# ChristophReich1996/Multi-StyleGAN

Measured on AMD Instinct MI355X. Metric: training images/sec (G+D step, 256^2, seq=3x2ch), higher is better.
Workload: dtype bf16

## Files before the change

### include/msg_hip.h

```cpp
#ifndef MSG_HIP_H
#define MSG_HIP_H

#ifdef __cplusplus
extern "C" {
#endif

enum { MSG_OK = 0, MSG_EINVAL = -1, MSG_EUNSUPPORTED = -2, MSG_ELAUNCH = -3 };
enum { MSG_F32 = 0, MSG_BF16 = 1, MSG_F16 = 2, MSG_F64 = 3, MSG_F32_SPLIT = 4 };

#define MSG_ABI_VERSION 5
int msg_abi_version(void);
const char* msg_build_arch(void);
const char* msg_strerror(int code);

int msg_upfirdn2d(const void* x, const float* fir, void* y, int dtype,
                  int major, int in_h, int in_w, int minor, int kh, int kw,
                  int up_x, int up_y, int down_x, int down_y,
                  int pad_x0, int pad_x1, int pad_y0, int pad_y1, void* stream);

int msg_upfirdn2d_pitched(const void* x, const float* fir, void* y, int dtype,
                          int major, int in_h, int in_w, int minor, int in_pitch, int kh, int kw,
                          int up_x, int up_y, int down_x, int down_y,
                          int pad_x0, int pad_x1, int pad_y0, int pad_y1, void* stream);

int msg_upfirdn2d_pitched2(const void* x, const float* fir, void* y, int dtype,
                           int major, int in_h, int in_w, int minor, int in_pitch, int out_pitch, int kh, int kw,
                           int up_x, int up_y, int down_x, int down_y,
                           int pad_x0, int pad_x1, int pad_y0, int pad_y1, void* stream);

int msg_upfirdn2d_separable(const void* x, const float* fir_y, const float* fir_x, void* y, int dtype,
                            int major, int in_h, int in_w, int minor, int kh, int kw,
                            int pad_x0, int pad_x1, int pad_y0, int pad_y1, void* stream);

int msg_upfirdn2d_separable_act(const void* x, const float* fir_y, const float* fir_x, void* y, int dtype,
                                int major, int in_h, int in_w, int minor, int kh, int kw,
                                int pad_x0, int pad_x1, int pad_y0, int pad_y1,
                                const float* act_bias, const float* noise, const float* noise_weight,
                                int noise_batch, float alpha, float scale, void* stream);
int msg_upfirdn2d_separable_act_mask(const void* x, const float* fir_y, const float* fir_x, void* y, int dtype,
                                     int major, int in_h, int in_w, int minor, int kh, int kw,
                                     int pad_x0, int pad_x1, int pad_y0, int pad_y1,
                                     const float* act_bias, const float* noise, const float* noise_weight,
                                     int noise_batch, float alpha, float scale, unsigned char* mask, void* stream);

int msg_fused_bias_act(const void* x, const float* bias, const void* ref, void* y, int dtype,
                       long long size_x, int step_b, int size_b,
                       const float* noise, const float* noise_weight, int noise_batch, int pix,
                       int act, int grad, float alpha, float scale, void* stream);

long long msg_bias_act_backward_workspace(long long size_x, int step_b, int size_b, int has_noise);
int msg_bias_act_backward(const void* gy, const void* out, void* gx, int dtype,
                          long long size_x, int step_b, int size_b,
                          float* grad_bias, const float* noise, float* grad_noise_weight,
                          int noise_batch, int pix, float alpha, float scale,
                          float* ws, long long ws_floats, void* stream);
int msg_channel_sums(const void* x, float* sums, int dtype, long long size_x, int C, float* ws, long long ws_floats,
                     void* stream);
int msg_bias_act_backward_mask(const void* gy, const unsigned char* mask, int tile_m, int tile_n, void* gx, int dtype,
                               long long size_x, int size_b,
                               float* grad_bias, const float* noise, float* grad_noise_weight,
                               int noise_batch, int pix, float alpha, float scale,
                               float* ws, long long ws_floats, void* stream);
int msg_sum_rows(const float* part, float* out, long long rows, int cols, void* stream);
int msg_bias_act_backward_mask_head(const void* gy, const void* ghead, const float* whead, const float* style,
                                    float wscale, int n_head, const unsigned char* mask, int tile_m, int tile_n,
                                    void* gx, int dtype, long long size_x, int size_b,
                                    float* grad_bias, const float* noise, float* grad_noise_weight,
                                    int noise_batch, int pix, float alpha, float scale,
                                    float* ws, long long ws_floats, void* stream);

int msg_conv2d_fprop(const void* x, const void* w, const float* bias, void* y, int dtype,
                     int B, int IH, int IW, int Cx, int Ck, int OH, int OW, int N, int ldy,
                     int kh, int kw, int stride, int pad, int in_up, int pixel_shuffle,
                     long long w_batch_stride, void* stream);
enum { MSG_WGRAD_K_AUTO = -1 };
int msg_conv2d_wgrad(const void* gy, const void* x, float* gw, int dtype,
                     int B, int IH, int IW, int Cx, int I, int OH, int OW, int ldgy, int O, int ldgw,
                     int kh, int kw, int stride, int pad, int pixel_shuffle,
                     int per_sample, int k_chunks, int oi_major, float gain,
                     float* ws, long long ws_floats, void* stream);
long long msg_conv2d_wgrad_workspace(int dtype, int B, int IH, int IW, int Cx, int I, int OH, int OW, int ldgy,
                                     int O, int ldgw, int kh, int kw, int stride, int pad, int pixel_shuffle,
                                     int per_sample, int k_chunks);

int msg_demod_coeff(const float* W, const float* s, float* d, int B, int O, int I, int taps,
                    float scale, float eps, void* stream);
int msg_scale_rows_cols(const float* base, const float* rowscale, const float* colscale, void* out,
                        int dtype, int B, int R, int T, int C, int Ck, float gain, void* stream);
int msg_modulate_weights(const float* base, const float* wsq, const float* style, void* out, float* d_out,
                         int dtype, int B, int R, int O, int T, int C, int Ck, float scale, float eps, void* stream);
int msg_modulate_backward(const float* gwk, const float* W, const float* s, const float* d, float* gW,
                          float* gs_part, int B, int O, int I, int taps, int ldg, int o_group,
                          float scale, void* stream);
int msg_scale_rows_cols2(const float* base, const float* row1, const float* col1, const float* row2, const float* col2,
                         void* out, int dtype, int B, int R, int T, int C, int Ck, float gain, void* stream);
int msg_modulate_backward2(const float* gwk, const float* W, const float* s, const float* d, const float* v,
                           float* gW, float* gs_part, int B, int O, int I, int taps, int ldg, int o_group,
                           float scale, void* stream);

int msg_relayout_weight(const float* w, void* fwd, void* dgrad, float* wsq, int dtype,
                        int O, int I, int T, int Ck, int Ok, int flip, int t_major, float gain, void* stream);

int msg_gather_taps(const void* x, void* y, int dtype, int B, int H, int W, int Cx, int C, int kh, int kw,
                    int pad, int Ko, void* stream);
int msg_fold_taps(const void* g, const void* add, void* gx, int dtype, int B, int H, int W, int Ko, int C, int kh, int kw,
                  int pad, int ldx, int ld_add, void* stream);

int msg_scaled_add(const void* a, const void* b, void* y, int dtype, long long n, float beta, float gain, void* stream);
int msg_rgb_skip_merge(const void* conv, int dtype, int ld, const float* bias, const float* skip, const float* fir,
                       float* out, int B, int C, int H, int W, void* stream);
int msg_rgb_skip_merge_backward(const float* g, void* g_conv, int dtype, int ld, float* g_skip, const float* fir,
                                int B, int C, int H, int W, void* stream);
int msg_gamma_merge(const void* a, const void* b, const float* gamma, void* y, int dtype, long long n, float gain, void* stream);
long long msg_gamma_merge_backward_workspace(void);
int msg_gamma_merge_backward(const void* gy, const void* a, const float* gamma, void* ga, void* gb, float* g_gamma, int dtype,
                             long long n, float gain, float* ws, void* stream);
int msg_scaled_add_rows(const void* a, const void* b, void* y, int dtype, long long rows, int cols,
                        long long lda, long long ldb, long long ldy, float beta, float gain, void* stream);

int msg_softmax_rows(const void* x, void* y, int dtype, long long rows, int cols, void* stream);
int msg_softmax_rows_backward(const void* y, const void* gy, void* gx, int dtype, long long rows, int cols,
                              void* stream);
int msg_softmax_rows_backward2(const void* y, const void* gy, const void* v, void* d_y, void* d_gy, int dtype,
                               long long rows, int cols, void* stream);

int msg_nonlocal_attention_supported(int B, int Nq, int Nk, int dk, int dv);
int msg_nonlocal_attention_fwd(const void* q, const void* k, const void* vt, void* o, float* lse, int dtype,
                               int B, int Nq, int Nk, int dk, int dv, void* stream);
int msg_maxpool2x2_fwd(const void* x, void* y, unsigned short* idx, int dtype, int B, int H, int W, int C, long long ldx,
                       void* stream);
int msg_maxpool2x2_bwd(const void* gy, const unsigned short* idx, void* gx, int dtype, int B, int H, int W, int C,
                       void* stream);
int msg_maxpool2x2_gather(const void* v, const unsigned short* idx, void* out, int dtype, int B, int H, int W, int C,
                          long long ldv, void* stream);

int msg_nonlocal_attention_bwd_splits(int B, int Nq, int Nk);
int msg_nonlocal_attention_bwd(const void* q, const void* qt, const void* k, const void* kt, const void* v,
                               const void* dO, const void* dOt, const void* o, const float* lse, float* delta,
                               void* dq, void* dk_out, void* dv_out, float* workspace, int dtype,
                               int B, int Nq, int Nk, int dk, int dv, void* stream);

int msg_affine_warp(const float* x, float* y, const float* angle_deg, float angle_const, const float* scale_xy,
                    const float* select_u, const float* p, int rot_prob, float cx, float cy, int padding,
                    int align_corners, int B, int C, int H, int W, int backward, void* workspace, void* stream);

long long msg_minibatch_stddev_workspace(int C, int H, int W, int groups, int dtype);
int msg_minibatch_stddev(const void* x, void* y, float* stat, float* workspace, int dtype,
                         int B, int C, int H, int W, int ldx, int ldy, int groups, float alpha, void* stream);
int msg_minibatch_stddev_backward(const void* x, const void* gy, const float* gstat, void* gx, int dtype,
                                  int B, int C, int H, int W, int ldx, int ldgy, int ldgx, int groups,
                                  float alpha, void* stream);

int msg_conv2d_fprop_act(const void* x, const void* w, void* y, int dtype,
                         int B, int IH, int IW, int Cx, int Ck, int OH, int OW, int N, int ldy,
                         int kh, int kw, int stride, int pad, long long w_batch_stride,
                         const float* act_bias, const float* noise, const float* noise_weight,
                         int noise_batch, float alpha, float scale, void* stream);
int msg_conv2d_fprop_act_mask(const void* x, const void* w, void* y, int dtype,
                              int B, int IH, int IW, int Cx, int Ck, int OH, int OW, int N, int ldy,
                              int kh, int kw, int stride, int pad, long long w_batch_stride,
                              const float* act_bias, const float* noise, const float* noise_weight,
                              int noise_batch, float alpha, float scale, unsigned char* mask, void* stream);

int msg_conv2d_fprop_residual(const void* x, const void* w, void* y, int dtype,
                              int B, int IH, int IW, int Cx, int Ck, int OH, int OW, int N, int ldy,
                              int kh, int kw, int stride, int pad, long long w_batch_stride,
                              const void* residual, int res_ld, float gain, void* stream);

int msg_conv2d_fprop_act_backward(const void* x, const void* w, void* y, int dtype,
                                  int B, int IH, int IW, int Cx, int Ck, int OH, int OW, int N, int ldy,
                                  int kh, int kw, int stride, int pad, long long w_batch_stride,
                                  const void* residual, int res_ld,
                                  const unsigned char* sign_mask, int mask_tile_m, int mask_tile_n,
                                  const void* sign_map, int sign_ld, float alpha, float scale,
                                  float* grad_bias, const float* noise, int noise_batch, float* grad_noise_weight,
                                  float* ws, long long ws_floats, void* stream);
// ... 116 lines not shown
```

### multi_stylegan_amd/conv_ops.py

```python
import ctypes
import functools
import math
import os
from typing import Optional, Tuple

import torch
from torch.autograd import Function

from . import _lib, weight_images
from ._autograd import _derive
from .weight_images import _k_run, _oi, _round_up
from .weight_images import invalidate_weight_cache


def _vec(dtype) -> int:
    return 8 if dtype == torch.bfloat16 else 4


def _padded_nhwc(b, c, h, w, dtype, device):
    cx = _round_up(c, _vec(dtype))
    buf = torch.empty((b, h, w, cx), dtype=dtype, device=device)
    if cx != c:
        buf[..., c:].zero_()
    return buf.permute(0, 3, 1, 2)[:, :c]
# ... 1107 lines not shown
    @staticmethod
    @torch.autograd.function.once_differentiable
    def backward(ctx, v):
        gy, *ws = ctx.saved_tensors
        slot, wscale, l = ctx.cfg
        g, dev = len(slot), gy.device
        gy, v = _dense32(gy, v)
        b, n, k = gy.shape[1], ws[0].shape[0], ws[0].shape[1]
        slot_t = _ptr_table_ints(slot, dev)
        d_gy, d_ws = None, [None] * g
        with _lib.on_device(dev):
            if ctx.needs_input_grad[0]:
                d_gy = torch.empty((g, b, n), dtype=torch.float32, device=dev)
                code = _lib.lib().msg_linear_grouped_fprop(v.data_ptr(), slot_t.data_ptr(), _ptr_table(ws, dev).data_ptr(), None,
                                                           d_gy.data_ptr(), g, b, n, k, l, wscale, 1.0, _lib.stream_of(dev))
                _lib.check(code, "msg_linear_grouped_fprop")
            if any(ctx.needs_input_grad[4:]):
                gw = torch.empty((g, n, k), dtype=torch.float32, device=dev)
                code = _lib.lib().msg_linear_grouped_wgrad(gy.data_ptr(), v.data_ptr(), slot_t.data_ptr(), gw.data_ptr(), None, g, b,
                                                           n, k, l, wscale, 1.0, _lib.stream_of(dev))
                _lib.check(code, "msg_linear_grouped_wgrad")
                d_ws = [gw[j] if ctx.needs_input_grad[4 + j] else None for j in range(g)]
        return (d_gy, None, None, None, *d_ws)


_INT_TABLES: dict = {}
_GATHER_TABLES: dict = {}


def _slot_gather_table(slot, n_slots, dev):
    key = (dev.index, tuple(int(v) for v in slot), n_slots)
    hit = _GATHER_TABLES.get(key)
    if hit is None:
        if len(_GATHER_TABLES) > 64:
            _GATHER_TABLES.clear()
        rows = [[j for j, v in enumerate(key[1]) if v == l] for l in range(n_slots)]
        width = max(1, max(len(r) for r in rows))
        hit = _GATHER_TABLES[key] = torch.tensor([r + [len(slot)] * (width - len(r)) for r in rows], dtype=torch.int64,
                                                 device=dev)
    return hit


def _ptr_table_ints(values, dev):
    key = (dev.index, tuple(int(v) for v in values))
    hit = _INT_TABLES.get(key)
    if hit is None:
        if len(_INT_TABLES) > 64:
            _INT_TABLES.clear()
        hit = _INT_TABLES[key] = torch.tensor(key[1], dtype=torch.int32, device=dev)
    return hit


def grouped_linear(latent, slots, weights, biases, wscale, bias_scale):
    return _GroupedLinear.apply(latent, tuple(int(v) for v in slots), float(wscale), float(bias_scale), *weights, *biases)


def demod_coefficients(weight, style, scale):
    wsq = weight[0].square().sum(dim=(2, 3))
    return torch.rsqrt((scale * scale) * (style.square() @ wsq.t()) + 1e-8)


def _modulated_composite(x, weight, style, demodulate, upsample):
    _, out_c, in_c, kh, kw = weight.shape
    scale = math.sqrt(2.0) / math.sqrt(in_c * kh * kw)
    coef = style[:, None, :] * scale
    if demodulate:
        coef = coef * demod_coefficients(weight, style, scale)[:, :, None]
    wmod = weight * coef[:, :, :, None, None]
    g = Geometry("up2" if upsample else "conv", kh, kw, 1, kh // 2, x.shape[2:], True)
    return _ConvF.apply(x, wmod, None, g)


def _scale_rows_cols(base, rowscale, colscale, out, gain):
    b, r, t, ck = out.shape
    c = base.shape[-1]
    dev = base.device
    with _lib.on_device(dev):
        code = _lib.lib().msg_scale_rows_cols(base.data_ptr(), _lib.ptr(rowscale), _lib.ptr(colscale), out.data_ptr(),
                                              _lib.dtype_code(out), b, r, t, c, ck, float(gain), _lib.stream_of(dev))
    _lib.check(code, "msg_scale_rows_cols")
    return out


_MODCONV_BWD_BATCH = 16


def _fold_weight_gradient(gwk, ldg, w3, s, dd, scale, style_dtype, cotangent=None, dest=None):
    b = gwk.shape[0]
    o, i, t = w3.shape
    dev = gwk.device
    og = 2 if o >= 512 or o < 256 else 1
    groups = (o + og - 1) // og
    out = _grad_dest(dest) if cotangent is None else None
    gw3 = out.view(o, i, t) if out is not None else torch.empty((o, i, t), dtype=torch.float32, device=dev)
    gs_part = _lib.scratch_ptr(groups * b * i, dev)
    gs = torch.empty((b, i), dtype=torch.float32, device=dev)
    with _lib.on_device(dev):
        st = _lib.stream_of(dev)
        if cotangent is None:
            code = _lib.lib().msg_modulate_backward(gwk.data_ptr(), w3.data_ptr(), s.data_ptr(), _lib.ptr(dd),
                                                    gw3.data_ptr(), gs_part, b, o, i, t, ldg, og, scale, st)
        else:
            code = _lib.lib().msg_modulate_backward2(gwk.data_ptr(), w3.data_ptr(), s.data_ptr(), _lib.ptr(dd),
                                                     cotangent.data_ptr(), gw3.data_ptr(), gs_part, b, o, i, t,
                                                     ldg, og, scale, st)
        _lib.check(code, "msg_modulate_backward" + ("2" if cotangent is not None else ""))
        code = _lib.lib().msg_sum_rows(gs_part, gs.data_ptr(), groups, b * i, st)
    _lib.check(code, "msg_sum_rows")
    return (out if out is not None else gw3), (gs if style_dtype == torch.float32 else gs.to(style_dtype))


def _modconv_backward(x, weight, style, d, gy, demodulate, upsample, g, scale, need, keep_gwk=False, direct=False,
                      act_bwd=None):
    _, o, i, kh, kw = weight.shape
    b, t = x.shape[0], kh * kw
    dev = x.device
    w3 = weight.detach().reshape(o, i, t)
    s = style.detach().float().contiguous()
    dd = d if demodulate else None
    gx = None
    if need[0]:
        okp = _round_up(o, _k_run(gy.dtype))
        wd = torch.empty((b, i, t, okp), dtype=gy.dtype, device=dev)
        base = weight_images.dgrad(weight, torch.float32, 1.0, g.kind, modulation=True)[0]
        _scale_rows_cols(base, s, dd, wd, scale)
        gx = _d_image(gy, wd, okp, o, i, g, act_bwd=act_bwd, sign_map=x)
    gw = gs = gwk = None
    if need[1] or need[2]:
        gwk, ldg = _g_raw(gy, x, o, i, g, raw=True)
        gw3, gs = _fold_weight_gradient(gwk, ldg, w3, s, dd, scale, style.dtype, dest=weight if direct else None)
        gw = gw3.reshape(1, o, i, kh, kw)
    return (gx, gw, gs, gwk) if keep_gwk else (gx, gw, gs)


_NATIVE_SECOND_ORDER = True


def _modconv_second_order_composite(gy, x, weight, style, demodulate, upsample, a, cot_w, cot_s, want):
    with torch.enable_grad():
        leaves = [t.detach().requires_grad_(True) for t in (gy, x, weight, style)]
        y2 = _modulated_composite(leaves[1], leaves[2], leaves[3], demodulate, upsample)
        first = torch.autograd.grad(y2, leaves[1:], leaves[0], create_graph=True, allow_unused=True)
        terms = [(c.to(f.dtype) * f).sum() for c, f in zip((a, cot_w, cot_s), first) if c is not None and f is not None]
        if not terms:
            return (None, None, None, None)
        grads = torch.autograd.grad(sum(terms), leaves, allow_unused=True)
    return tuple(gr if w else None for gr, w in zip(grads, want))


class _ModConvGrad(Function):

    @staticmethod
    def forward(ctx, gy, x, weight, style, d, demodulate, upsample, g, scale, need):
        gx, gw, gs, gwk = _modconv_backward(x, weight, style, d, gy, demodulate, upsample, g, scale, need, keep_gwk=True)
        ctx.set_materialize_grads(False)
        ctx.save_for_backward(gy, x, weight, style, d, gwk)
        ctx.cfg = (demodulate, upsample, g, scale)
        return gx, gw, gs

    @staticmethod
    @torch.autograd.function.once_differentiable
    def backward(ctx, a, cot_w, cot_s):
        gy, x, weight, style, d, gwk = ctx.saved_tensors
        demodulate, upsample, g, scale = ctx.cfg
        want = ctx.needs_input_grad[:4]
        _, o, i, kh, kw = weight.shape
        b, t = x.shape[0], kh * kw
        tail = (None,) * 6
        if a is None and cot_w is None and cot_s is None:
            return (None, None, None, None) + tail
        if cot_w is not None or i % 4 or i > 512 or t not in (1, 4, 9) or b > _MODCONV_BWD_BATCH or \
                (cot_s is not None and gwk is None):
            return _modconv_second_order_composite(gy, x, weight, style, demodulate, upsample, a, cot_w, cot_s, want) + tail
        dev = x.device
        w3 = weight.detach().reshape(o, i, t)
        s = style.detach().float().contiguous()
        dd = d if demodulate else None
        ck, okp = _round_up(i, _k_run(gy.dtype)), _round_up(o, _k_run(gy.dtype))
        rows = t * o if upsample else o
        ggy = gx2 = gw3 = gs2 = None
        if a is not None:
            a = a.to(x.dtype)
            if want[0]:
                wk = torch.empty((b, rows, 1 if upsample else t, ck), dtype=x.dtype, device=dev)
                base = weight_images.forward(weight, torch.float32, 1.0, g.kind, modulation=True)[0]
                _scale_rows_cols(base, (d.repeat(1, t) if upsample else d) if demodulate else None, s, wk, scale)
                ggy = _f_image(a, wk, ck, o, i, g)
            if want[2] or want[3]:
                gwk_a, ldg = _g_raw(gy, a, o, i, g, raw=True)
                gw3, gs2 = _fold_weight_gradient(gwk_a, ldg, w3, s, dd, scale, style.dtype)
        if cot_s is not None:
            v = cot_s.detach().float().contiguous()
            if want[0] or want[1]:
                hf = torch.empty((b, rows, 1 if upsample else t, ck), dtype=x.dtype, device=dev)
                hd = torch.empty((b, i, t, okp), dtype=gy.dtype, device=dev)
                base_f = weight_images.forward(weight, torch.float32, 1.0, g.kind, modulation=True)[0]
                base_d = weight_images.dgrad(weight, torch.float32, 1.0, g.kind, modulation=True)[0]
                if demodulate:
                    wsq = weight_images.tap_square_sums(weight, g.kind)
                    ddir = -(scale * scale) * d.pow(3) * linear(s * v, wsq)
                    rows_d, rows_dd = (d.repeat(1, t), ddir.repeat(1, t)) if upsample else (d, ddir)
                    with _lib.on_device(dev):
                        lib, st = _lib.lib(), _lib.stream_of(dev)
                        code = lib.msg_scale_rows_cols2(base_f.data_ptr(), rows_d.contiguous().data_ptr(), v.data_ptr(),
                                                        rows_dd.contiguous().data_ptr(), s.data_ptr(), hf.data_ptr(),
                                                        _lib.dtype_code(hf), b, rows, 1 if upsample else t, i, ck, scale, st)
                        _lib.check(code, "msg_scale_rows_cols2")
                        code = lib.msg_scale_rows_cols2(base_d.data_ptr(), v.data_ptr(), d.data_ptr(), s.data_ptr(),
                                                        ddir.contiguous().data_ptr(), hd.data_ptr(), _lib.dtype_code(hd), b, i, t,
                                                        o, okp, scale, st)
                        _lib.check(code, "msg_scale_rows_cols2")
                else:
                    _scale_rows_cols(base_f, None, v, hf, scale)
                    _scale_rows_cols(base_d, v, None, hd, scale)
                if want[0]:
                    ggy = _f_image(x, hf, ck, o, i, g, residual=None if ggy is None else (ggy, 1.0))
                if want[1]:
                    gx2 = _d_image(gy, hd, okp, o, i, g)
            if want[2] or want[3]:
                gw3b, gs2b = _fold_weight_gradient(gwk, gwk.shape[-1], w3, s, dd, scale, style.dtype, cotangent=v)
                gw3 = gw3b if gw3 is None else gw3 + gw3b
                gs2 = gs2b if gs2 is None else gs2 + gs2b
        gw = gw3.reshape(1, o, i, kh, kw) if (gw3 is not None and want[2]) else None
        return (ggy, gx2, gw, gs2 if want[3] else None) + tail


class _ModulatedConv(Function):

    @staticmethod
    def forward(ctx, x, weight, style, demodulate, upsample, act_bias=None, noise=None, noise_w=None, alpha=0.2,
                act_scale=1.0, fuse_act=False, head_slot=None, input_act=None):
        dev = _lib.require_gpu(x, weight, style)
        ctx.input_act = input_act if input_act is not None and input_act.armed else None
        ctx.head_slot = head_slot
        if head_slot is not None and fuse_act:
            ctx.set_materialize_grads(False)
            head_slot.armed = True
        _, o, i, kh, kw = weight.shape
        b, t = x.shape[0], kh * kw
        scale = math.sqrt(2.0) / math.sqrt(i * t)
        s = style.detach().float().contiguous()
        d = None
        ck = _round_up(i, _k_run(x.dtype))
        kind = "up2" if upsample else "conv"
        base = weight_images.forward(weight, torch.float32, 1.0, kind, modulation=True)[0]
        rows = t * o if upsample else o
        wk = torch.empty((b, rows, 1 if upsample else t, ck), dtype=x.dtype, device=dev)
        if demodulate:
            wsq = weight_images.tap_square_sums(weight, kind)
            d = torch.empty((b, o), dtype=torch.float32, device=dev)
            with _lib.on_device(dev):
                code = _lib.lib().msg_modulate_weights(base.data_ptr(), wsq.data_ptr(), s.data_ptr(), wk.data_ptr(),
                                                       d.data_ptr(), _lib.dtype_code(wk), b, rows, o,
                                                       1 if upsample else t, i, ck, scale, 1e-8, _lib.stream_of(dev))
            _lib.check(code, "msg_modulate_weights")
        else:
            _scale_rows_cols(base, None, s, wk, scale)
        g = Geometry(kind, kh, kw, 1, kh // 2, x.shape[2:], True)
        act = None
        holder = [] if any(ctx.needs_input_grad) else None
        if fuse_act:
            assert not upsample, "the upsampling layers blur before their activation"
            act = (*_act_operands(act_bias, noise, noise_w, (b, o, *g.y_hw)), alpha, act_scale, holder)
        y = _f_image(x, wk, ck, o, i, g, act=act)
        ctx.save_for_backward(x, weight, style, d if d is not None else torch.empty(0, device=dev),
                              y if fuse_act else None, noise if fuse_act else None)
        ctx.cfg = (demodulate, upsample, g, scale)
        ctx.act = (alpha, act_scale, act_bias is not None, noise is not None,
                   None if noise_w is None else noise_w.shape) if fuse_act else None
        ctx.bias_param = act_bias
        ctx.mask = holder[0] if holder else None
        return y

    @staticmethod
    def backward(ctx, gy):
        x, weight, style, d, y_act, noise = ctx.saved_tensors
        demodulate, upsample, g, scale = ctx.cfg
        _, o, i, kh, kw = weight.shape
        b, t = x.shape[0], kh * kw
        need = list(ctx.needs_input_grad)
        need[1], need[2] = _consumed(ctx, 1, 1), _consumed(ctx, 2, 2)
        gb = gnw = None
        slot = ctx.head_slot
        if ctx.act is not None:
            from .op_static.fused_act import FusedLeakyReLUFunctionBackward, act_backward_with_head
            alpha, act_scale, has_bias, has_noise, nw_shape = ctx.act
            head, head_dgrad = slot.take() if slot is not None else (None, None)
            fused = None
            if head is not None:
                fused = act_backward_with_head(gy, head, y_act.shape, noise if has_noise else None,
                                               ctx.bias_param if has_bias else None, has_bias, alpha, act_scale, ctx.mask)
                if fused is None:
                    gh = head_dgrad()
                    gy = gh if gy is None else gy + gh
            if fused is not None:
                gy, gb, gnw = fused
            elif gy is None:
                return (None,) * 13
            else:
                gy, gb, gnw = _derive(FusedLeakyReLUFunctionBackward, gy, y_act, noise if has_noise else None,
                                      ctx.bias_param if has_bias else False, alpha, act_scale, ctx.mask)
            gb = gb if has_bias and need[5] else None
            gnw = gnw.reshape(nw_shape) if has_noise and need[7] else None
        tail = (None, None, gb, None, gnw, None, None, None, None, None)
        if ctx.act is None and slot is not None and slot.armed and need[0] and not torch.is_grad_enabled() and \
                fused_head_ok(gy, weight, b, demodulate, upsample):
            gyc, wt, st = gy, weight, style
            slot.head = (gyc, weight.detach().reshape(o, i).float().contiguous(), style.detach().float().contiguous(), scale)
            slot.dgrad = lambda: _modconv_backward(x, wt, st, d, gyc, demodulate, upsample, g, scale,
                                                   [True, False, False])[0]
            need[0] = False
        fused_ok = i <= 512 and t <= 9
        if torch.is_grad_enabled() and fused_ok and _NATIVE_SECOND_ORDER and b <= _MODCONV_BWD_BATCH and x.is_cuda:
            gx, gw, gs = _derive(_ModConvGrad, gy, x, weight, style, d if demodulate else None, demodulate, upsample, g, scale,
                                            tuple(need[:3]))
            return (gx, gw, gs) + tail
        if torch.is_grad_enabled() or not fused_ok:
            with torch.enable_grad():
                ins = [v for v, n in zip((x, weight, style), need[:3]) if n]
                y2 = _modulated_composite(x, weight, style, demodulate, upsample)
                grads = list(torch.autograd.grad(y2, ins, gy, create_graph=torch.is_grad_enabled(), allow_unused=True))
            out = [grads.pop(0) if n else None for n in need[:3]]
            return (out[0], out[1], out[2]) + tail
        if b > _MODCONV_BWD_BATCH:
            gxs, gws, gss = [], [], []
            for lo in range(0, b, _MODCONV_BWD_BATCH):
                hi = min(b, lo + _MODCONV_BWD_BATCH)
                cgx, cgw, cgs = _modconv_backward(x[lo:hi], weight, style[lo:hi], d[lo:hi] if demodulate else d,
                                                  gy[lo:hi], demodulate, upsample, g, scale, need)
                gxs.append(cgx); gws.append(cgw); gss.append(cgs)
            gx = torch.cat(gxs) if need[0] else None
            gw = torch.stack(gws).sum(dim=0) if gws[0] is not None else None
            gs = torch.cat(gss) if gss[0] is not None else None
            return (gx, gw, gs) + tail
        gx, gw, gs = _modconv_backward(x, weight, style, d, gy, demodulate, upsample, g, scale, need, direct=True,
                                       act_bwd=ctx.input_act)
        return (gx, gw, gs) + tail


def fused_head_ok(gy, weight, b, demodulate, upsample) -> bool:
    _, o, _, kh, kw = weight.shape
    return gy is not None and gy.is_cuda and gy.dtype == torch.bfloat16 and kh == 1 and kw == 1 and o <= 8 and \
        not demodulate and not upsample and b <= _MODCONV_BWD_BATCH and HEAD_GRAD_FUSION


HEAD_GRAD_FUSION = bool(int(os.environ.get("MSG_HEAD_GRAD_FUSION", "1")))

# ... 13 lines not shown
```

### multi_stylegan_amd/csrc/modulate.hip

```cpp
#include "msg_common.h"
#include <stdlib.h>

__device__ __forceinline__ float block_sum_256(float v, float* red ) {
    v = wave_sum(v);
    __syncthreads();
    if ((threadIdx.x & 63) == 0) red[threadIdx.x >> 6] = v;
    __syncthreads();
    return red[0] + red[1] + red[2] + red[3];
}

__global__ __launch_bounds__(256) void demod_coeff_kernel(const float* __restrict__ W, const float* __restrict__ s,
                                                          float* __restrict__ d, int B, int O, int I, int T,
                                                          float scale, float eps) {
    __shared__ float red[4];
    const int o = blockIdx.x;
    const float* wo = W + (size_t)o * I * T;
    for (int b = 0; b < B; ++b) {
        float acc = 0.f;
        for (int i = threadIdx.x; i < I; i += 256) {
            const float sv = s[(size_t)b * I + i];
            float w2 = 0.f;
            for (int t = 0; t < T; ++t) { const float wv = wo[i * T + t]; w2 = fmaf(wv, wv, w2); }
            acc = fmaf(w2, sv * sv, acc);
        }
// ... 131 lines not shown
            for (int b = b0; b < b1; ++b) {
                const float rs1 = gain * row1[(size_t)b * R + r], rs2 = gain * row2[(size_t)b * R + r];
                float sc[VEC], s2[VEC];
                load_run<VEC>(col1 + (size_t)b * C, c0, C, al, sc);
                load_run<VEC>(col2 + (size_t)b * C, c0, C, al, s2);
#pragma unroll
                for (int e = 0; e < VEC; ++e) sc[e] = fmaf(rs1, sc[e], rs2 * s2[e]);
                TO* dst_row = out + ((size_t)b * R + r) * T * Ck;
#pragma unroll
                for (int k = 0; k < SRC_ITEMS; ++k) {
                    const int t = tb + k * tstep;
                    if (t >= T) break;
                    V o;
                    if constexpr (VEC == 4) {
#pragma unroll
                        for (int e = 0; e < 4; ++e) o.set(e, f[k][e] * sc[e]);
                    } else {
#pragma unroll
                        for (int e = 0; e < 4; ++e) o.set2(e, f[k][2 * e] * sc[2 * e], f[k][2 * e + 1] * sc[2 * e + 1]);
                    }
                    *reinterpret_cast<uint4*>(dst_row + (size_t)t * Ck + c0) = o.raw;
                }
            }
        }
    }
}

extern "C" int msg_scale_rows_cols2(const float* base, const float* row1, const float* col1, const float* row2,
                                    const float* col2, void* out, int dtype, int B, int R, int T, int C, int Ck, float gain,
                                    void* stream) {
    if (B == 0) return MSG_OK;
    if (!base || !row1 || !col1 || !row2 || !col2 || !out || B < 0 || R <= 0 || T <= 0 || C <= 0 || Ck < C) return MSG_EINVAL;
    if (dtype != MSG_F32 && dtype != MSG_BF16) return MSG_EUNSUPPORTED;
    const int vec = dtype == MSG_BF16 ? 8 : 4;
    if (Ck % vec || (((uintptr_t)out) & 15u)) return MSG_EUNSUPPORTED;
    hipStream_t s = (hipStream_t)stream;
    int bg = 1;
    while (bg < 8 && bg * 2 <= B && (long long)R * ((B + 2 * bg - 1) / (2 * bg)) >= 2048) bg *= 2;
    dim3 grid(R, (B + bg - 1) / bg);
    if (dtype == MSG_BF16)
        hipLaunchKernelGGL((scale_rows_cols2_kernel<bf16_t>), grid, dim3(256), 0, s, base, row1, col1, row2, col2,
                           (bf16_t*)out, B, bg, R, T, C, Ck, gain);
    else
        hipLaunchKernelGGL((scale_rows_cols2_kernel<float>), grid, dim3(256), 0, s, base, row1, col1, row2, col2,
                           (float*)out, B, bg, R, T, C, Ck, gain);
    return MSG_CHECK_LAUNCH();
}

template <typename TO>
__global__ __launch_bounds__(256) void modulate_weights_kernel(const float* __restrict__ base, const float* __restrict__ wsq,
                                                               const float* __restrict__ style, TO* __restrict__ out,
                                                               float* __restrict__ d_out, int B, int BG, int R, int O,
                                                               int T, int C, int Ck, float scale, float eps) {
    using V = Vec16<TO>;
    constexpr int VEC = V::N;
    __shared__ float red[4 * 8];
    __shared__ float dsh[8];
    const int o = blockIdx.x, b0 = blockIdx.y * BG, b1 = min(B, b0 + BG);
    {
        float part[8];
#pragma unroll
        for (int k = 0; k < 8; ++k) part[k] = 0.f;
        for (int i = threadIdx.x; i < C; i += 256) {
            const float q = wsq[(size_t)o * C + i];
#pragma unroll
            for (int k = 0; k < 8; ++k)
                if (b0 + k < b1) { const float sv = style[(size_t)(b0 + k) * C + i]; part[k] = fmaf(q, sv * sv, part[k]); }
        }
#pragma unroll
        for (int k = 0; k < 8; ++k) {
            const float v = wave_sum(part[k]);
            if ((threadIdx.x & 63) == 0) red[(threadIdx.x >> 6) * 8 + k] = v;
        }
        __syncthreads();
        if (threadIdx.x < 8 && b0 + (int)threadIdx.x < b1) {
            const int k = threadIdx.x;
            const float tot = red[k] + red[8 + k] + red[16 + k] + red[24 + k];
            const float dv = rsqrtf(scale * scale * tot + eps);
            dsh[k] = dv;
            if (d_out) d_out[(size_t)(b0 + k) * O + o] = dv;
        }
        __syncthreads();
    }
    const int cvecs = Ck / VEC;
    const int tstep = 256 / cvecs > 0 ? 256 / cvecs : 1;
    const bool al = (C % 4 == 0) && ((((uintptr_t)base | (uintptr_t)style) & 15u) == 0);
    const int npairs = (R / O) * T;
    for (int cv = threadIdx.x % cvecs; cv < cvecs; cv += 256) {
        const int c0 = cv * VEC;
        const int t0 = threadIdx.x / cvecs;
        for (int qb = t0; qb < npairs; qb += tstep * SRC_ITEMS) {
            float f[SRC_ITEMS][VEC];
            size_t cell[SRC_ITEMS];
#pragma unroll
            for (int k = 0; k < SRC_ITEMS; ++k) {
                const int q = qb + k * tstep;
                const int rk = q / T, t = q - rk * T;
                cell[k] = (size_t)(o + rk * O) * T + t;
                if (q < npairs) load_run<VEC>(base + cell[k] * C, c0, C, al, f[k]);
                else {
#pragma unroll
                    for (int e = 0; e < VEC; ++e) f[k][e] = 0.f;
                }
            }
            for (int b = b0; b < b1; ++b) {
                const float rs = scale * dsh[b - b0];
                float sc[VEC];
                load_run<VEC>(style + (size_t)b * C, c0, C, al, sc);
#pragma unroll
                for (int e = 0; e < VEC; ++e) sc[e] *= rs;
                TO* dst_b = out + (size_t)b * R * T * Ck;
#pragma unroll
                for (int k = 0; k < SRC_ITEMS; ++k) {
                    if (qb + k * tstep >= npairs) break;
                    V ov;
                    if constexpr (VEC == 4) {
#pragma unroll
                        for (int e = 0; e < 4; ++e) ov.set(e, f[k][e] * sc[e]);
                    } else {
#pragma unroll
                        for (int e = 0; e < 4; ++e) ov.set2(e, f[k][2 * e] * sc[2 * e], f[k][2 * e + 1] * sc[2 * e + 1]);
                    }
                    *reinterpret_cast<uint4*>(dst_b + cell[k] * Ck + c0) = ov.raw;
                }
            }
        }
    }
}

extern "C" int msg_modulate_weights(const float* base, const float* wsq, const float* style, void* out, float* d_out,
                                    int dtype, int B, int R, int O, int T, int C, int Ck, float scale, float eps,
                                    void* stream) {
    if (B == 0) return MSG_OK;
    if (!base || !wsq || !style || !out || B < 0 || R <= 0 || O <= 0 || R % O || T <= 0 || C <= 0 || Ck < C) return MSG_EINVAL;
    if (dtype != MSG_F32 && dtype != MSG_BF16) return MSG_EUNSUPPORTED;
    const int vec = dtype == MSG_BF16 ? 8 : 4;
    if (Ck % vec || ((uintptr_t)out & 15u) || B > 65535) return MSG_EUNSUPPORTED;
    hipStream_t s = (hipStream_t)stream;
    static const int min_wgs = msg_tunable("MSG_MODW_MIN_WGS", 1024);
    int bg = 1;
    while (bg < 8 && bg * 2 <= B && (long long)O * ((B + 2 * bg - 1) / (2 * bg)) >= min_wgs) bg *= 2;
    dim3 grid(O, (B + bg - 1) / bg);
    if (dtype == MSG_BF16)
        hipLaunchKernelGGL((modulate_weights_kernel<bf16_t>), grid, dim3(256), 0, s, base, wsq, style, (bf16_t*)out, d_out,
                           B, bg, R, O, T, C, Ck, scale, eps);
    else
        hipLaunchKernelGGL((modulate_weights_kernel<float>), grid, dim3(256), 0, s, base, wsq, style, (float*)out, d_out,
                           B, bg, R, O, T, C, Ck, scale, eps);
    return MSG_CHECK_LAUNCH();
}

constexpr int MB_SLOTS = 2;
constexpr int MB_TAPS = 9;
constexpr int MB_BMAX = 32;
template <bool DEMOD>
__global__ __launch_bounds__(256) void modulate_backward_kernel(const float* __restrict__ gwk, const float* __restrict__ W,
                                                                const float* __restrict__ s, const float* __restrict__ d,
                                                                float* __restrict__ gW, float* __restrict__ gs_part,
                                                                int B, int O, int I, int T, int ldg, int OG, float scale) {
    __shared__ float red[4 * MB_BMAX];
    __shared__ float Tsh[MB_BMAX];
    const int og = blockIdx.x;
    const int tid = threadIdx.x, lane = tid & 63, wid = tid >> 6;
    float gs_acc[MB_BMAX / 2][MB_SLOTS];
#pragma unroll
    for (int b = 0; b < MB_BMAX / 2; ++b)
#pragma unroll
        for (int k = 0; k < MB_SLOTS; ++k) gs_acc[b][k] = 0.f;

    for (int oo = 0; oo < OG; ++oo) {
        const int o = og * OG + oo;
        if (o >= O) break;
        float wv[MB_SLOTS][MB_TAPS], gacc[MB_SLOTS][MB_TAPS];
#pragma unroll
        for (int k = 0; k < MB_SLOTS; ++k) {
            const int i = tid + 256 * k;
#pragma unroll
            for (int t = 0; t < MB_TAPS; ++t) {
                wv[k][t] = (i < I && t < T) ? W[((size_t)o * I + i) * T + t] : 0.f;
                gacc[k][t] = 0.f;
            }
        }
        if (DEMOD) {
            for (int b = 0; b < B; ++b) {
                float part = 0.f;
#pragma unroll
                for (int k = 0; k < MB_SLOTS; ++k) {
                    const int i = tid + 256 * k;
                    if (i >= I) continue;
                    const float sv = s[(size_t)b * I + i];
                    const float* g = gwk + (((size_t)b * O + o) * T) * ldg + i;
#pragma unroll
                    for (int t = 0; t < MB_TAPS; ++t)
                        if (t < T) part = fmaf(g[(size_t)t * ldg], wv[k][t] * sv, part);
                }
                part = wave_sum(part);
                if (lane == 0) red[wid * MB_BMAX + b] = part;
            }
            __syncthreads();
            if (tid < B) Tsh[tid] = scale * (red[tid] + red[MB_BMAX + tid] + red[2 * MB_BMAX + tid] + red[3 * MB_BMAX + tid]);
            __syncthreads();
        }
#pragma unroll
        for (int b = 0; b < MB_BMAX / 2; ++b) {
            if (b >= B) break;
            const float dv = DEMOD ? d[(size_t)b * O + o] : 1.f;
            const float corr = DEMOD ? dv * dv * dv * Tsh[b] : 0.f;
#pragma unroll
            for (int k = 0; k < MB_SLOTS; ++k) {
                const int i = tid + 256 * k;
                if (i >= I) continue;
                const float sv = s[(size_t)b * I + i];
                const float* g = gwk + (((size_t)b * O + o) * T) * ldg + i;
                float sgrad = 0.f;
#pragma unroll
                for (int t = 0; t < MB_TAPS; ++t) {
                    if (t >= T) continue;
                    const float gu = dv * g[(size_t)t * ldg] - corr * (scale * wv[k][t] * sv);
                    gacc[k][t] = fmaf(gu, sv, gacc[k][t]);
                    sgrad = fmaf(gu, wv[k][t], sgrad);
                }
                gs_acc[b][k] += sgrad;
            }
        }
#pragma unroll
        for (int k = 0; k < MB_SLOTS; ++k) {
            const int i = tid + 256 * k;
            if (i >= I) continue;
#pragma unroll
            for (int t = 0; t < MB_TAPS; ++t)
                if (t < T) gW[((size_t)o * I + i) * T + t] = scale * gacc[k][t];
        }
        if (DEMOD) __syncthreads();
    }
// ... 350 lines not shown
```

Before: 157.5.

## Fuse weight modulation into MFMA conv kernel for small-resolution modulated convs

Adds a dedicated small-spatial (at most 64 pixels) modulated conv kernel that loads the fp32 base weights, applies per-sample row and column scales on the fly, and feeds bf16 MFMA directly. This avoids materializing a per-sample modulated weight tensor and launching a separate modulation kernel for the low-resolution layers. It is used in both forward and the input-gradient path, with a separate demod-coefficient-only launch. The risk is that a one-wave-per-block kernel has low occupancy, and the new path adds eligibility logic and more code to maintain.

```diff
diff --git a/include/msg_hip.h b/include/msg_hip.h
--- a/include/msg_hip.h
+++ b/include/msg_hip.h
@@ -92,6 +92,16 @@
 int msg_modulate_backward(const float* gwk, const float* W, const float* s, const float* d, float* gW,
                           float* gs_part, int B, int O, int I, int taps, int ldg, int o_group,
                           float scale, void* stream);
+int msg_demod_coeff_wsq(const float* wsq, const float* style, float* d_out, int B, int O, int C, float scale,
+                        float eps, void* stream);
+int msg_conv2d_small_mod_eligible(int dtype, int B, int IH, int IW, int Cx, int C, int OH, int OW, int R, int ldy,
+                                  int kh, int kw, int stride, int pad, int in_up, int pixel_shuffle, int per_sample,
+                                  int epilogue);
+int msg_conv2d_small_mod(const void* x, const float* base, const float* rowscale, const float* colscale, int row_mod,
+                         float gain, void* y, int dtype, int B, int IH, int IW, int Cx, int C, int OH, int OW, int R,
+                         int ldy, int kh, int kw, int stride, int pad, int in_up, int pixel_shuffle,
+                         const float* act_bias, const float* noise, const float* noise_weight, int noise_batch,
+                         float alpha, float scale, int epilogue, void* stream);
 int msg_scale_rows_cols2(const float* base, const float* row1, const float* col1, const float* row2, const float* col2,
                          void* out, int dtype, int B, int R, int T, int C, int Ck, float gain, void* stream);
 int msg_modulate_backward2(const float* gwk, const float* W, const float* s, const float* d, const float* v,
diff --git a/multi_stylegan_amd/conv_ops.py b/multi_stylegan_amd/conv_ops.py
--- a/multi_stylegan_amd/conv_ops.py
+++ b/multi_stylegan_amd/conv_ops.py
@@ -1213,6 +1213,50 @@
     return out
 
 
+SMALL_MODCONV = bool(int(os.environ.get("MSG_SMALL_MODCONV", "1")))
+
+
+def _small_modconv(x, base, n, out_hw, kh, kw, stride, pad, in_up, pixel_shuffle, c_real, act=None):
+    if not SMALL_MODCONV or not x.is_cuda:
+        return None
+    dev = x.device
+    b, _, ih, iw = x.shape
+    oh, ow = out_hw
+    c = base.shape[-1]
+    code_x = _lib.dtype_code(x)
+    epilogue = int(act is not None)
+    ldy = _round_up(n // 4 if pixel_shuffle else n, _vec(x.dtype))
+    xv, cx = _nhwc_view(x)
+    geom = (code_x, b, ih, iw, cx, c, oh, ow, n, ldy, kh, kw, stride, pad, in_up, int(pixel_shuffle))
+    if not _lib.lib().msg_conv2d_small_mod_eligible(*geom, 1, epilogue):
+        return None
+
+    def launch(rowscale, colscale, row_mod, gain):
+        if pixel_shuffle:
+            y, ld = _alloc_out(b, n // 4, 2 * oh, 2 * ow, x.dtype, dev)
+        else:
+            y, ld = _alloc_out(b, n, oh, ow, x.dtype, dev)
+        assert ld == ldy
+        act_bias = noise = noise_w = None
+        alpha = scale = 0.0
+        if act is not None:
+            act_bias, noise, noise_w, alpha, scale = act[:5]
+            _lib.require_gpu(x, act_bias, noise, noise_w)
+        key = "conv_fprop_small"
+        if _lib.kernel_clock.enabled and _CLOCK_SHAPES:
+            key += _shape_key(b, (ih, iw), out_hw, c_real, n, kh, kw, stride,
+                              f" up{in_up}{' ps' if pixel_shuffle else ''} per-sample")
+        flops = 2.0 * b * oh * ow * n * kh * kw * c_real / (in_up * in_up)
+        with _lib.on_device(dev), _lib.kernel_clock.span((key, 'bf16'), flops):
+            code = _lib.lib().msg_conv2d_small_mod(
+                xv.data_ptr(), base.data_ptr(), _lib.ptr(rowscale), _lib.ptr(colscale), int(row_mod), float(gain), y.data_ptr(),
+                *geom, _lib.ptr(act_bias), _lib.ptr(noise), _lib.ptr(noise_w), 1 if noise is None else noise.shape[0],
+                float(alpha), float(scale), epilogue, _lib.stream_of(dev))
+        _lib.check(code, "msg_conv2d_small_mod")
+        return y
+    return launch
+
+
 _MODCONV_BWD_BATCH = 16
 
 
@@ -1251,11 +1295,16 @@
     dd = d if demodulate else None
     gx = None
     if need[0]:
-        okp = _round_up(o, _k_run(gy.dtype))
-        wd = torch.empty((b, i, t, okp), dtype=gy.dtype, device=dev)
         base = weight_images.dgrad(weight, torch.float32, 1.0, g.kind, modulation=True)[0]
-        _scale_rows_cols(base, s, dd, wd, scale)
-        gx = _d_image(gy, wd, okp, o, i, g, act_bwd=act_bwd, sign_map=x)
+        small = _small_modconv(gy, base, i, g.x_hw, 2, 2, 2, 0, 1, False, o) if g.kind == "up2" else \
+            _small_modconv(gy, base, i, g.x_hw, g.kh, g.kw, 1, g.kh - 1 - g.pad, g.stride, False, o)
+        if small is not None:
+            gx = small(s, dd, i, scale)
+        else:
+            okp = _round_up(o, _k_run(gy.dtype))
+            wd = torch.empty((b, i, t, okp), dtype=gy.dtype, device=dev)
+            _scale_rows_cols(base, s, dd, wd, scale)
+            gx = _d_image(gy, wd, okp, o, i, g, act_bwd=act_bwd, sign_map=x)
     gw = gs = gwk = None
     if need[1] or need[2]:
         gwk, ldg = _g_raw(gy, x, o, i, g, raw=True)
@@ -1376,24 +1425,36 @@
         kind = "up2" if upsample else "conv"
         base = weight_images.forward(weight, torch.float32, 1.0, kind, modulation=True)[0]
         rows = t * o if upsample else o
-        wk = torch.empty((b, rows, 1 if upsample else t, ck), dtype=x.dtype, device=dev)
-        if demodulate:
-            wsq = weight_images.tap_square_sums(weight, kind)
-            d = torch.empty((b, o), dtype=torch.float32, device=dev)
-            with _lib.on_device(dev):
-                code = _lib.lib().msg_modulate_weights(base.data_ptr(), wsq.data_ptr(), s.data_ptr(), wk.data_ptr(),
-                                                       d.data_ptr(), _lib.dtype_code(wk), b, rows, o,
-                                                       1 if upsample else t, i, ck, scale, 1e-8, _lib.stream_of(dev))
-            _lib.check(code, "msg_modulate_weights")
-        else:
-            _scale_rows_cols(base, None, s, wk, scale)
         g = Geometry(kind, kh, kw, 1, kh // 2, x.shape[2:], True)
         act = None
         holder = [] if any(ctx.needs_input_grad) else None
         if fuse_act:
             assert not upsample, "the upsampling layers blur before their activation"
             act = (*_act_operands(act_bias, noise, noise_w, (b, o, *g.y_hw)), alpha, act_scale, holder)
-        y = _f_image(x, wk, ck, o, i, g, act=act)
+        small = _small_modconv(x, base, 4 * o, g.x_hw, 1, 1, 1, 0, 1, True, i) if upsample else \
+            _small_modconv(x, base, o, g.y_hw, kh, kw, g.stride, g.pad, 1, False, i, act=act)
+        if small is not None:
+            if demodulate:
+                wsq = weight_images.tap_square_sums(weight, kind)
+                d = torch.empty((b, o), dtype=torch.float32, device=dev)
+                with _lib.on_device(dev):
+                    code = _lib.lib().msg_demod_coeff_wsq(wsq.data_ptr(), s.data_ptr(), d.data_ptr(), b, o, i, scale, 1e-8,
+                                                          _lib.stream_of(dev))
+                _lib.check(code, "msg_demod_coeff_wsq")
+            y = small(d, s, o, scale)
+        else:
+            wk = torch.empty((b, rows, 1 if upsample else t, ck), dtype=x.dtype, device=dev)
+            if demodulate:
+                wsq = weight_images.tap_square_sums(weight, kind)
+                d = torch.empty((b, o), dtype=torch.float32, device=dev)
+                with _lib.on_device(dev):
+                    code = _lib.lib().msg_modulate_weights(base.data_ptr(), wsq.data_ptr(), s.data_ptr(), wk.data_ptr(),
+                                                           d.data_ptr(), _lib.dtype_code(wk), b, rows, o,
+                                                           1 if upsample else t, i, ck, scale, 1e-8, _lib.stream_of(dev))
+                _lib.check(code, "msg_modulate_weights")
+            else:
+                _scale_rows_cols(base, None, s, wk, scale)
+            y = _f_image(x, wk, ck, o, i, g, act=act)
         ctx.save_for_backward(x, weight, style, d if d is not None else torch.empty(0, device=dev),
                               y if fuse_act else None, noise if fuse_act else None)
         ctx.cfg = (demodulate, upsample, g, scale)
diff --git a/multi_stylegan_amd/csrc/conv_small_mod.hip b/multi_stylegan_amd/csrc/conv_small_mod.hip
--- /dev/null
+++ b/multi_stylegan_amd/csrc/conv_small_mod.hip
@@ -0,0 +1,270 @@
+#include "msg_common.h"
+
+typedef __bf16 sm_bf16v8 __attribute__((ext_vector_type(8)));
+typedef __bf16 sm_bf16v2 __attribute__((ext_vector_type(2)));
+typedef float sm_f32v2 __attribute__((ext_vector_type(2)));
+
+constexpr int SM_NT = 32;
+constexpr int SM_MAX_PIX = 64;
+constexpr int SM_MAX_CK = 512;
+constexpr int SM_DEPTH = 4;
+constexpr int SM_ROWB = SM_MAX_CK * 2 + 16;
+constexpr int SM_SCROW = SM_MAX_CK + 4;
+struct SmallModParams {
+    int B, H, W, Cx, C, Ck, R, ldy, T, kw, pad, pixel_shuffle, row_mod;
+    float gain;
+    ActEpilogue act;
+};
+
+__device__ __forceinline__ unsigned sm_pack2(float lo, float hi) {
+    return __builtin_bit_cast(unsigned, __builtin_convertvector(sm_f32v2{lo, hi}, sm_bf16v2));
+}
+
+template <int MT, bool TABLE, bool RAGGED>
+__global__ __launch_bounds__(64) void conv_small_mod_kernel(const bf16_t* __restrict__ x, const float* __restrict__ base,
+                                                            const float* __restrict__ rowscale, const float* __restrict__ colscale,
+                                                            bf16_t* __restrict__ y, SmallModParams p) {
+    __shared__ __attribute__((aligned(16))) char xs[(SM_MAX_PIX + 1) * SM_ROWB];
+    __shared__ __attribute__((aligned(16))) float scs[TABLE ? SM_NT * SM_SCROW : SM_MAX_CK];
+    __shared__ float rsv[SM_NT];
+    const int lane = threadIdx.x, lr = lane & 31, lh = lane >> 5;
+    const int n0 = blockIdx.x * SM_NT, b = blockIdx.y;
+    const int hw = p.H * p.W, n_chunks = p.Ck >> 6, nks = p.T * n_chunks;
+    const int nsub = p.pixel_shuffle ? 4 : 1, sub_rows = p.R / nsub;
+
+    int oh[MT], ow[MT];
+    bool pok[MT];
+#pragma unroll
+    for (int mt = 0; mt < MT; ++mt) {
+        const int pix = mt * 32 + lr;
+        pok[mt] = pix < hw;
+        const int pp = pok[mt] ? pix : 0;
+        oh[mt] = pp / p.W;
+        ow[mt] = pp - oh[mt] * p.W;
+    }
+
+    for (int sub = 0; sub < nsub; ++sub) {
+        const int r = sub * sub_rows + n0 + lr;
+        const float rs = p.gain * (rowscale ? rowscale[(size_t)b * p.row_mod + r % p.row_mod] : 1.f);
+        const float* wrow = base + (size_t)r * p.T * p.C + lh * 8;
+
+        f32x4 wq[SM_DEPTH][8];
+        int ld_t = 0, ld_c = 0;
+        const float* wptr = wrow;
+        auto issue = [&](f32x4 (&dst)[8]) __attribute__((always_inline)) {
+            if constexpr (RAGGED) {
+                const float* src = wrow + (size_t)ld_t * p.C + ld_c * 64;
+#pragma unroll
+                for (int kk = 0; kk < 4; ++kk) {
+                    const bool ok = ld_c * 64 + kk * 16 + lh * 8 + 8 <= p.C;
+                    const f32x4* q = reinterpret_cast<const f32x4*>(ok ? src + kk * 16 : base);
+                    dst[2 * kk] = q[0];
+                    dst[2 * kk + 1] = q[1];
+                }
+                if (++ld_c == n_chunks) { ld_c = 0; ++ld_t; }
+            } else {
+                const f32x4* q = reinterpret_cast<const f32x4*>(wptr);
+#pragma unroll
+                for (int kk = 0; kk < 4; ++kk) {
+                    dst[2 * kk] = q[4 * kk];
+                    dst[2 * kk + 1] = q[4 * kk + 1];
+                }
+                wptr += 64;
+            }
+        };
+#pragma unroll
+        for (int s = 0; s < SM_DEPTH; ++s)
+            if (s < nks) issue(wq[s]);
+
+        __syncthreads();
+        if (TABLE && lane < SM_NT) rsv[lane] = rs;
+        if (sub == 0) {
+            const int cvecs = p.Ck >> 3, xvecs = p.Cx >> 3, total = hw * cvecs;
+            const uint4* xb = reinterpret_cast<const uint4*>(x + (size_t)b * hw * p.Cx);
+            for (int v0 = 0; v0 < total; v0 += 64 * 8) {
+                uint4 tmp[8];
+                int dst[8];
+#pragma unroll
+                for (int u = 0; u < 8; ++u) {
+                    const int v = v0 + u * 64 + lane;
+                    const int pix = v / cvecs, cv = v - pix * cvecs;
+                    dst[u] = v < total ? pix * SM_ROWB + cv * 16 : -1;
+                    tmp[u] = (v < total && cv < xvecs) ? xb[(size_t)pix * xvecs + cv] : make_uint4(0, 0, 0, 0);
+                }
+#pragma unroll
+                for (int u = 0; u < 8; ++u)
+                    if (dst[u] >= 0) *reinterpret_cast<uint4*>(xs + dst[u]) = tmp[u];
+            }
+            for (int cv = lane; cv < cvecs; cv += 64)
+                *reinterpret_cast<uint4*>(xs + SM_MAX_PIX * SM_ROWB + cv * 16) = make_uint4(0, 0, 0, 0);
+            if (!TABLE)
+                for (int c = lane; c < p.Ck; c += 64)
+                    scs[c] = c < p.C ? (colscale ? colscale[(size_t)b * p.C + c] : 1.f) : 0.f;
+        }
+        if constexpr (TABLE) {
+            __syncthreads();
+            const int c4s = p.Ck >> 2;
+            for (int v = lane; v < SM_NT * c4s; v += 64) {
+                const int row = v / c4s, c = (v - row * c4s) * 4;
+                f32x4 cv = {0.f, 0.f, 0.f, 0.f};
+                if (c < p.C) {
+                    if (colscale) cv = *reinterpret_cast<const f32x4*>(colscale + (size_t)b * p.C + c);
+                    else cv = f32x4{1.f, 1.f, 1.f, 1.f};
+                }
+                const float rr = rsv[row];
+#pragma unroll
+                for (int e = 0; e < 4; ++e) cv[e] *= rr;
+                *reinterpret_cast<f32x4*>(scs + row * SM_SCROW + c) = cv;
+            }
+        }
+        __syncthreads();
+
+        f32x16 acc[MT];
+#pragma unroll
+        for (int mt = 0; mt < MT; ++mt)
+#pragma unroll
+            for (int e = 0; e < 16; ++e) acc[mt][e] = 0.f;
+
+        int cp_c = 0, th = 0, tw = 0;
+        int xoff[MT];
+        auto set_tap = [&]() __attribute__((always_inline)) {
+#pragma unroll
+            for (int mt = 0; mt < MT; ++mt) {
+                const int ih = oh[mt] + th - p.pad, iw = ow[mt] + tw - p.pad;
+                const bool ok = pok[mt] & ((unsigned)ih < (unsigned)p.H) & ((unsigned)iw < (unsigned)p.W);
+                xoff[mt] = (ok ? ih * p.W + iw : SM_MAX_PIX) * SM_ROWB + lh * 16;
+            }
+        };
+        set_tap();
+        auto compute = [&](const f32x4 (&wv)[8]) __attribute__((always_inline)) {
+            const float* sp = scs + (TABLE ? lr * SM_SCROW : 0) + cp_c * 64 + lh * 8;
+#pragma unroll
+            for (int kk = 0; kk < 4; ++kk) {
+                const f32x4 f0 = wv[2 * kk], f1 = wv[2 * kk + 1];
+                f32x4 s0 = *reinterpret_cast<const f32x4*>(sp + kk * 16), s1 = *reinterpret_cast<const f32x4*>(sp + kk * 16 + 4);
+                if constexpr (!TABLE) {
+#pragma unroll
+                    for (int e = 0; e < 4; ++e) { s0[e] *= rs; s1[e] *= rs; }
+                }
+                u32x4 wp;
+                wp[0] = sm_pack2(f0[0] * s0[0], f0[1] * s0[1]);
+                wp[1] = sm_pack2(f0[2] * s0[2], f0[3] * s0[3]);
+                wp[2] = sm_pack2(f1[0] * s1[0], f1[1] * s1[1]);
+                wp[3] = sm_pack2(f1[2] * s1[2], f1[3] * s1[3]);
+                if constexpr (RAGGED) {
+                    if (cp_c * 64 + kk * 16 + lh * 8 + 8 > p.C) wp = u32x4{0u, 0u, 0u, 0u};
+                }
+                const sm_bf16v8 wf = __builtin_bit_cast(sm_bf16v8, wp);
+#pragma unroll
+                for (int mt = 0; mt < MT; ++mt) {
+                    const u32x4 xv = *reinterpret_cast<const u32x4*>(xs + xoff[mt] + cp_c * 128 + kk * 32);
+                    acc[mt] = __builtin_amdgcn_mfma_f32_32x32x16_bf16(wf, __builtin_bit_cast(sm_bf16v8, xv), acc[mt], 0, 0, 0);
+                }
+            }
+            if (++cp_c == n_chunks) {
+                cp_c = 0;
+                if (++tw == p.kw) { tw = 0; ++th; }
+                set_tap();
+            }
+        };
+        int ks0 = 0;
+        for (; ks0 + 2 * SM_DEPTH <= nks; ks0 += SM_DEPTH) {
+#pragma unroll
+            for (int s = 0; s < SM_DEPTH; ++s) {
+                compute(wq[s]);
+                issue(wq[s]);
+            }
+        }
+#pragma unroll
+        for (int s = 0; s < SM_DEPTH; ++s) {
+            if (ks0 + s < nks) {
+                compute(wq[s]);
+                if (ks0 + s + SM_DEPTH < nks) issue(wq[s]);
+            }
+        }
+#pragma unroll
+        for (int s = 0; s < SM_DEPTH; ++s)
+            if (ks0 + SM_DEPTH + s < nks) compute(wq[s]);
+
+        const bool want_act = p.act.enabled == 1;
+        const bool want_noise = want_act && p.act.noise;
+        const float nw = want_noise ? p.act.noise_w[0] : 0.f;
+#pragma unroll
+        for (int mt = 0; mt < MT; ++mt) {
+            if (!pok[mt]) continue;
+            const int pix = mt * 32 + lr;
+            const long long gp = p.pixel_shuffle
+                ? ((long long)(b * 2 * p.H + 2 * oh[mt] + (sub >> 1)) * (2 * p.W) + 2 * ow[mt] + (sub & 1))
+                : (long long)b * hw + pix;
+            const float nv = want_noise ? nw * p.act.noise[(long long)(p.act.noise_batch == 1 ? 0 : b) * hw + pix] : 0.f;
+            bf16_t* dst = y + gp * p.ldy + n0 + 4 * lh;
+#pragma unroll
+            for (int g = 0; g < 4; ++g) {
+                uint2 pk;
+                pk.x = (unsigned)f2bf(acc[mt][4 * g + 0] + 0.f) | ((unsigned)f2bf(acc[mt][4 * g + 1] + 0.f) << 16);
+                pk.y = (unsigned)f2bf(acc[mt][4 * g + 2] + 0.f) | ((unsigned)f2bf(acc[mt][4 * g + 3] + 0.f) << 16);
+                if (want_act) {
+                    float bv[8];
+#pragma unroll
+                    for (int e = 0; e < 8; ++e) bv[e] = (e < 4 && p.act.bias) ? p.act.bias[n0 + 8 * g + 4 * lh + e] : 0.f;
+                    const u32x4 o = act_epilogue_apply<bf16_t>(u32x4{pk.x, pk.y, 0u, 0u}, bv, nv, p.act.alpha, p.act.scale);
+                    pk.x = o[0]; pk.y = o[1];
+                }
+                *reinterpret_cast<uint2*>(dst + 8 * g) = pk;
+            }
+        }
+    }
+}
+
+extern "C" int msg_conv2d_small_mod_eligible(int dtype, int B, int IH, int IW, int Cx, int C, int OH, int OW, int R, int ldy,
+                                             int kh, int kw, int stride, int pad, int in_up, int pixel_shuffle, int per_sample,
+                                             int epilogue) {
+    static const int enabled = msg_tunable("MSG_CONV_SMALL_MOD", 1);
+    if (!enabled || dtype != MSG_BF16 || !per_sample || B <= 0 || B > 65535) return 0;
+    if (IH <= 0 || IW <= 0 || IH != OH || IW != OW || (long long)IH * IW > SM_MAX_PIX) return 0;
+    if (stride != 1 || in_up != 1 || kh != kw) return 0;
+    if (!((kh == 3 && pad == 1 && !pixel_shuffle) || (kh == 1 && pad == 0))) return 0;
+    if (epilogue != 0 && (epilogue != 1 || pixel_shuffle)) return 0;
+    if (C <= 0 || C % 8 || Cx < C || Cx % 8 || (C + 63) / 64 * 64 > SM_MAX_CK || Cx > SM_MAX_CK) return 0;
+    if (R <= 0 || R % SM_NT || R / SM_NT > 65535) return 0;
+    if (pixel_shuffle ? (R % 4 || (R / 4) % SM_NT || ldy < R / 4) : ldy < R) return 0;
+    if (ldy % 4) return 0;
+    return 1;
+}
+
+template <int MT, bool TABLE>
+static void small_mod_launch(bool ragged, dim3 grid, hipStream_t st, const bf16_t* x, const float* base, const float* rowscale,
+                             const float* colscale, bf16_t* y, const SmallModParams& p) {
+    if (ragged) hipLaunchKernelGGL((conv_small_mod_kernel<MT, TABLE, true>), grid, dim3(64), 0, st, x, base, rowscale, colscale, y, p);
+    else hipLaunchKernelGGL((conv_small_mod_kernel<MT, TABLE, false>), grid, dim3(64), 0, st, x, base, rowscale, colscale, y, p);
+}
+
+extern "C" int msg_conv2d_small_mod(const void* x, const float* base, const float* rowscale, const float* colscale, int row_mod,
+                                    float gain, void* y, int dtype, int B, int IH, int IW, int Cx, int C, int OH, int OW, int R,
+                                    int ldy, int kh, int kw, int stride, int pad, int in_up, int pixel_shuffle,
+                                    const float* act_bias, const float* noise, const float* noise_weight, int noise_batch,
+                                    float alpha, float scale, int epilogue, void* stream) {
+    if (B == 0) return MSG_OK;
+    if (!x || !base || !y || row_mod <= 0 || (rowscale && R % row_mod)) return MSG_EINVAL;
+    if (epilogue == 1 && noise && (!noise_weight || (noise_batch != 1 && noise_batch != B))) return MSG_EINVAL;
+    if (!msg_conv2d_small_mod_eligible(dtype, B, IH, IW, Cx, C, OH, OW, R, ldy, kh, kw, stride, pad, in_up, pixel_shuffle, 1, epilogue))
+        return MSG_EUNSUPPORTED;
+    if ((((uintptr_t)x | (uintptr_t)base | (uintptr_t)colscale) & 15u) || (((uintptr_t)y) & 7u)) return MSG_EUNSUPPORTED;
+    SmallModParams p{};
+    p.B = B; p.H = IH; p.W = IW; p.Cx = Cx; p.C = C; p.Ck = (C + 63) / 64 * 64; p.R = R; p.ldy = ldy;
+    p.T = kh * kw; p.kw = kw; p.pad = pad; p.pixel_shuffle = pixel_shuffle; p.row_mod = row_mod; p.gain = gain;
+    if (epilogue == 1) p.act = ActEpilogue{act_bias, noise, noise_weight, noise_batch, 1, alpha, scale, nullptr, 0, 0.f, nullptr};
+    const dim3 grid((pixel_shuffle ? R / 4 : R) / SM_NT, B);
+    const bool ragged = C % 64 != 0, one_tile = IH * IW <= 32;
+    const hipStream_t st = (hipStream_t)stream;
+    const bf16_t* xp = (const bf16_t*)x;
+    bf16_t* yp = (bf16_t*)y;
+    if (p.T > 1) {
+        if (one_tile) small_mod_launch<1, true>(ragged, grid, st, xp, base, rowscale, colscale, yp, p);
+        else small_mod_launch<2, true>(ragged, grid, st, xp, base, rowscale, colscale, yp, p);
+    } else {
+        if (one_tile) small_mod_launch<1, false>(ragged, grid, st, xp, base, rowscale, colscale, yp, p);
+        else small_mod_launch<2, false>(ragged, grid, st, xp, base, rowscale, colscale, yp, p);
+    }
+    return MSG_CHECK_LAUNCH();
+}
diff --git a/multi_stylegan_amd/csrc/modulate.hip b/multi_stylegan_amd/csrc/modulate.hip
--- a/multi_stylegan_amd/csrc/modulate.hip
+++ b/multi_stylegan_amd/csrc/modulate.hip
@@ -237,6 +237,7 @@
         }
         __syncthreads();
     }
+    if (!out) return;
     const int cvecs = Ck / VEC;
     const int tstep = 256 / cvecs > 0 ? 256 / cvecs : 1;
     const bool al = (C % 4 == 0) && ((((uintptr_t)base | (uintptr_t)style) & 15u) == 0);
@@ -305,6 +306,17 @@
     return MSG_CHECK_LAUNCH();
 }
 
+extern "C" int msg_demod_coeff_wsq(const float* wsq, const float* style, float* d_out, int B, int O, int C, float scale,
+                                   float eps, void* stream) {
+    if (B == 0) return MSG_OK;
+    if (!wsq || !style || !d_out || B < 0 || O <= 0 || C <= 0) return MSG_EINVAL;
+    if (B > 8 * 65535) return MSG_EUNSUPPORTED;
+    const int bg = B >= 8 ? 8 : B;
+    hipLaunchKernelGGL((modulate_weights_kernel<bf16_t>), dim3(O, (B + bg - 1) / bg), dim3(256), 0, (hipStream_t)stream,
+                       (const float*)nullptr, wsq, style, (bf16_t*)nullptr, d_out, B, bg, O, O, 1, C, C, scale, eps);
+    return MSG_CHECK_LAUNCH();
+}
+
 constexpr int MB_SLOTS = 2;
 constexpr int MB_TAPS = 9;
 constexpr int MB_BMAX = 32;
```

Result: no change. 157.8, median of 2 (+0.1%).
